# AdaptiveCity/deepdish

Measured on AMD Instinct MI355X. Metric: end-to-end frames/sec (detect+encode+track) at 640x480, higher is better.
Workload: dtype i8 (reference: uint8); encoder f16; 1 GPU; SSD-MobileNet-v1 uint8-quantised (300x300) + MARS-64x32x3 + deep_sort on synthetic 640x480 BGR frames, ~20 synthetic detections/frame (BASELINE.json configs[1]); streams_per_gpu=3072, worker_threads_per_gpu=2, parallelism=independent streams, 3072 per GPU in 2 worker groups, weights=seeded synthetic (seed 1234)

## Files before the change

deepdish_amd/build.py:

```python
import os
import subprocess
import sys
from concurrent.futures import ThreadPoolExecutor

HERE = os.path.dirname(os.path.abspath(__file__))
CSRC = os.path.join(HERE, 'csrc')
OBJ = os.path.join(CSRC, '_obj')
LIB = os.path.join(HERE, 'libdeepdish_hip.so')
HIPCC = os.environ.get('HIPCC', '/opt/rocm/bin/hipcc')
ARCH = 'gfx950'

COMMON = ['--offload-arch=' + ARCH, '-O3', '-fPIC', '-std=c++17', '-Wall', '-Wno-unused-function',
          '-I', os.path.join(HERE, '..', 'include')]
STRICT_FP = {'kalman.hip', 'cost.hip', 'nms.hip', 'tracker.hip', 'lsap.cpp', 'pyset.cpp', 'api.hip', 'image.hip', 'pipeline.hip', 'mog2.hip', 'post.hip'}


EXTRA = ({'netsq.hip': ['-mllvm', '-amdgpu-mfma-vgpr-form'], 'netsq_front.hip': ['-mllvm', '-amdgpu-mfma-vgpr-form'], 'netsq_mid.hip': ['-mllvm', '-amdgpu-mfma-vgpr-form'], 'mars_tail.hip': ['-mllvm', '-amdgpu-mfma-vgpr-form'],
          'mars_pair.hip': ['-mllvm', '-amdgpu-mfma-vgpr-form']}
         if os.environ.get('DD_NO_VGPR_FORM') != '1' else {})


def _sources():
    return sorted(f for f in os.listdir(CSRC) if f.endswith(('.hip', '.cpp')))


def _headers_mtime():
    hs = [os.path.join(CSRC, f) for f in os.listdir(CSRC) if f.endswith('.h')]
    hs.append(os.path.join(HERE, '..', 'include', 'deepdish_hip.h'))
    return max(os.path.getmtime(h) for h in hs)


def _compile(src, force, hmt):
    obj = os.path.join(OBJ, src + '.o')
    path = os.path.join(CSRC, src)
    if (not force and os.path.exists(obj)
            and os.path.getmtime(obj) >= max(os.path.getmtime(path), hmt, os.path.getmtime(__file__))):
        return obj, False
    cmd = [HIPCC] + COMMON + (['-ffp-contract=off'] if src in STRICT_FP else []) + EXTRA.get(src, []) + ['-x', 'hip', '-c', path, '-o', obj]
    r = subprocess.run(cmd, capture_output=True, text=True)
    if r.returncode != 0:
# ... 27 lines not shown
```

deepdish_amd/csrc/net_priv.h:

```cpp
#pragma once
#include <map>
#include <utility>
#include <vector>
#include "common.h"

struct TensorDesc { int buf, h, w, c, cs, coff, dtype, pad; };

struct dd_net {
    dd_ctx *ctx = nullptr;
    int max_batch = 0;
    std::vector<int32_t> prog;
    std::vector<TensorDesc> tensors;
    std::vector<int64_t> buf_elems;
    std::vector<void *> bufs;
    std::vector<int> buf_dtype;
    int n_ops = 0, ops_off = 0;
    void *arena = nullptr;
    int64_t arena_bytes = 0;
    char *d_weights = nullptr;
    int64_t weight_bytes = 0;
    int in_h = 0, in_w = 0, out_tensor = -1;
    bool profile = false;
    int last_batch = 0;
    DevBuf slab;
    bool ssd_dec = false, yolo_dec = false;
    int dec_anchors = 0; float dec_thr = 0.f;
    float *d_anchors = nullptr, *dec_boxes = nullptr, *dec_score = nullptr, *dec_keys = nullptr; int *dec_cls = nullptr;
    bool slab_moved = false;
    _Float16 *d_zero = nullptr;
    bool use_glds = true;
    bool use_rw = true;
    int tile_mode = 0;
    std::vector<hipEvent_t> events;
    std::vector<int32_t> op_launch;
    struct GraphEntry { int calls = 0; hipGraph_t graph = nullptr; hipGraphExec_t exec = nullptr; };
    bool use_graph = false;
    std::map<std::pair<const void *, int>, GraphEntry> graphs;
};

int netq_run_op(dd_net *net, int op_index, const int32_t *o, const uint8_t *input, int nimg, hipStream_t s, int *handled);
int netq_run_front(dd_net *net, const int32_t *o0, const int32_t *o1, const int32_t *o2, const uint8_t *input, int nimg, hipStream_t s, int *ran);
int netq_run_mid(dd_net *net, const int32_t *o3, const int32_t *o4, int nimg, hipStream_t s, int *ran);
int netq_prepare(dd_net *net);
```

deepdish_amd/csrc/nets.hip:

```cpp
#include <algorithm>
#include <cmath>
#include <cstdlib>
#include <map>
#include <string>
#include "common.h"
#include "ssd_dev.h"
#include "net_priv.h"
#include "mars_tail.h"

namespace {

typedef _Float16 h8 __attribute__((ext_vector_type(8)));
typedef _Float16 h4 __attribute__((ext_vector_type(4)));
typedef float f4 __attribute__((ext_vector_type(4)));

enum { OP_INPUT = 1, OP_CONV = 2, OP_DWCONV = 3, OP_MAXPOOL = 4, OP_UPSAMPLE = 5, OP_FC = 6, OP_L2NORM = 7, OP_STEM = 8, OP_DWPW = 9 };
enum { ACT_NONE = 0, ACT_RELU6 = 1, ACT_ELU = 2, ACT_SILU = 3, ACT_RELU = 4, ACT_SIGMOID = 5 };
enum { EPI_F16 = 0, EPI_F32 = 1, EPI_SSD_HEAD = 2, EPI_YOLO = 3 };
enum { OPK_DEFAULT = 0, OPK_FOLDED = 1, OPK_POOL_ROWS = 2, OPK_POOL_ROWS_STEM = 3, OPK_RES_UNIT = 4, OPK_SSD_FRONT = 5, OPK_C64_ROWS = 6, OPK_S2_ROWS = 7, OPK_CONV_WS = 8, OPK_WS_DW = 9, OPK_DWPW_ROWS = 10, OPK_SSD_HEAD_DEC = 11, OPK_RES_PAIR = 12, OPK_YOLO_HEAD_DEC = 13, OPK_MARS_WS = 14, OPK_FOLDED_PREV = 15, OPK_MARS_PAIR = 16, OPK_C64_STRIPS = 18, OPK_Q_FRONT = 19, OPK_Q_MID = 20, OPK_STEM_WIDE = 23 };
enum { DT_F16 = 0, DT_F32 = 1, DT_U8 = 2 };

constexpr int OP_WORDS = 48;
constexpr int TENSOR_WORDS = 8;

__device__ __forceinline__ float fast_sigmoid(float v) { return __builtin_amdgcn_rcpf(1.f + __expf(-v)); }

__device__ __forceinline__ float yolo_box_col(int o, float s, float px, float py, float stride, float aw, float ah, float img_w, float img_h) {
#pragma clang fp contract(off)
    if (o == 0) return (s * 2.f - 0.5f + px) * stride / img_w;
    if (o == 1) return (s * 2.f - 0.5f + py) * stride / img_h;
    if (o == 2) return (s * 2.f) * (s * 2.f) * aw / img_w;
    return (s * 2.f) * (s * 2.f) * ah / img_h;
}

__device__ __forceinline__ float apply_act(float v, int act) {
    switch (act) {
        case ACT_RELU6: return __builtin_amdgcn_fmed3f(v, 0.f, 6.f);
        case ACT_ELU: {
            float e = __builtin_amdgcn_exp2f(v * 1.44269504088896340736f);
            e = __builtin_amdgcn_fmed3f(e, 0.f, 1.f);
            return __builtin_amdgcn_fmed3f(v, e - 1.f, 3.0e38f);
        }
        case ACT_SILU: {
            float r = v * fast_sigmoid(v);
#if defined(__HIP_DEVICE_COMPILE__)
// ... 4324 lines not shown
    bool stem_pending = false;
    bool wide_pending = false, wide_ready = false;
    bool input_pending = false;
    float input_mean = 0.f, input_scale = 1.f;
    int input_op = -1;
    ConvP unit_a;
    bool unit_pending = false;
    ConvP pw_p;
    bool pw_pending = false;
    bool proj_done = false;
    MarsPairP pair64;
    bool pair64_first = false;
    int pair_left = 0;
    ConvP pair_a, pair_b;
    bool pair_pending = false;
    int pair_op = -1;
    auto flush_pair = [&]() -> int {
        pair_pending = false;
        net->op_launch[pair_op] = OPK_RES_UNIT;
        return launch_res_unit(s, pair_a, pair_b, nimg, net->ctx->device);
    };
    auto run_ws = [&](ConvP &P) { return P.cin == 256 ? launch_conv_ws<4>(s, P, net->ctx->device) : launch_conv_ws<8>(s, P, net->ctx->device); };
    int first_op = 0;
    bool mid_on = false;
    {
        static const int chunk_env = getenv("DD_Q_FRONT_CHUNK") ? atoi(getenv("DD_Q_FRONT_CHUNK")) : 0;
        auto opw = [&](int k) { return net->prog.data() + net->ops_off + (size_t)k * OP_WORDS; };
        const char *front_env = getenv("DD_Q_FRONT"), *front_min_env = getenv("DD_Q_FRONT_MIN");
        const int front_min = front_min_env ? atoi(front_min_env) : 24;
        {
            const char *mid_env = getenv("DD_Q_MID");
            mid_on = !(mid_env && atoi(mid_env) == 0) && nimg >= front_min;
        }
        if (!(front_env && atoi(front_env) == 0) && chunk_env <= 0 && nimg >= front_min && net->n_ops > 3 && opw(0)[0] == 16 && opw(1)[0] == 19 && opw(2)[0] == 19) {
            if (net->profile) for (int k = 0; k < 3; ++k) DD_HIP(hipEventRecord(net->events[k], s));
            int ran = 0;
            const int rc = netq_run_front(net, opw(0), opw(1), opw(2), input, nimg, s, &ran);
            if (rc != DD_OK) return rc;
            if (ran) { first_op = 3; net->op_launch[0] = OPK_FOLDED; net->op_launch[1] = OPK_FOLDED; net->op_launch[2] = OPK_Q_FRONT; }
        }
        if (first_op == 0 && chunk_env > 0 && nimg > chunk_env && net->n_ops > 3 && opw(0)[0] == 16 && opw(1)[0] == 19 && opw(2)[0] == 19 && opw(1)[1] == opw(0)[2] && opw(2)[1] == opw(1)[2]) {
            const TensorDesc &t2 = net->tensors[opw(2)[2]];
            const size_t img_out = (size_t)(t2.h + 2) * (t2.w + 2) * t2.cs;
            void *&out_buf = net->bufs[t2.buf];
            void *const out_base = out_buf;
            if (net->profile) for (int k = 0; k < 3; ++k) DD_HIP(hipEventRecord(net->events[k], s));
            for (int c0 = 0; c0 < nimg; c0 += chunk_env) {
                const int nc = std::min(chunk_env, nimg - c0);
                out_buf = static_cast<char *>(out_base) + (size_t)c0 * img_out;
                for (int k = 0; k < 3; ++k) {
                    int handled = 0;
                    const int rc = netq_run_op(net, k, opw(k), input + (size_t)c0 * net->in_h * net->in_w * 3, nc, s, &handled);
                    if (rc != DD_OK || !handled) { out_buf = out_base; return rc != DD_OK ? rc : DD_E_ARG; }
                }
            }
            out_buf = out_base;
            first_op = 3;
        }
    }
    for (int i = first_op; i < net->n_ops; ++i) {
        if (net->profile) DD_HIP(hipEventRecord(net->events[i], s));
        const int32_t *o = net->prog.data() + net->ops_off + (size_t)i * OP_WORDS;
        const float *of = reinterpret_cast<const float *>(o);
        const int kind = o[0], src = o[1], dst = o[2], res = o[3], dst2 = o[4];
        const TensorDesc *ts = src >= 0 ? &net->tensors[src] : nullptr;
        const TensorDesc *td = dst >= 0 ? &net->tensors[dst] : nullptr;
        DD_REQUIRE(!input_pending || (kind == OP_CONV && i == input_op + 1), DD_E_STATE, "dd_net_forward: input op %d was folded into an op that did not take it", input_op);
        if (mid_on && kind == 19 && i + 1 < net->n_ops && net->prog[net->ops_off + (size_t)(i + 1) * OP_WORDS] == 19) {
            const int32_t *o4 = net->prog.data() + net->ops_off + (size_t)(i + 1) * OP_WORDS;
            if (net->profile) DD_HIP(hipEventRecord(net->events[i + 1], s));
            int ran = 0;
            const int rc = netq_run_mid(net, o, o4, nimg, s, &ran);
            if (rc != DD_OK) return rc;
            if (ran) { net->op_launch[i] = OPK_FOLDED; net->op_launch[i + 1] = OPK_Q_MID; ++i; continue; }
        }
        DD_REQUIRE((!wide_pending || kind == OP_CONV) && (!wide_ready || kind == OP_MAXPOOL), DD_E_STATE, "dd_net_forward: op %d does not take the first layer folded into it", i);
        if (pair_pending && kind != OP_CONV) { const int rc = flush_pair(); if (rc != DD_OK) return rc; }
        if (pw_pending && kind != OP_DWCONV) {
            pw_pending = false; net->op_launch[i - 1] = OPK_CONV_WS;
            const int rc = run_ws(pw_p);
            if (rc != DD_OK) return rc;
        }
        if (unit_pending && kind != OP_CONV) {
            unit_pending = false; net->op_launch[i - 1] = OPK_DEFAULT;
            const int rc = launch_conv3x3_rw(s, unit_a, nimg, false, net->ctx->device);
            if (rc != DD_OK) return rc;
        }
        if (stem_pending && !(kind == OP_CONV && o[29]) && kind != OP_DWPW) {
            stem_pending = false; net->op_launch[i - 1] = OPK_DEFAULT;
            const int rc = launch_stem(s, stem_p, nimg);
            if (rc != DD_OK) return rc;
        }
        switch (kind) {
            case OP_INPUT: {
                const int s2d = o[5];
                const int m = nimg * td->h * td->w;
                if (s2d && o[30] && !o[6] && td->cs == 32 && !td->coff && i + 1 < net->n_ops && net->use_rw) {
// ... 403 lines not shown
```

deepdish_amd/csrc/netsq_front.hip:

```cpp
#include <algorithm>
#include <atomic>
#include <cstdlib>
#include <type_traits>
#include "common.h"
#include "net_priv.h"
#include "netsq_dev.h"

namespace {

constexpr int F_S0 = 300, F_S1 = 150, F_S2 = 75;
constexpr int F_PP = (F_S1 + 2) * 16;
constexpr int F_RB0 = 2 * F_PP, F_RB1 = 4 * F_PP;
constexpr int F_NR0 = 4, F_NR1 = 3;
constexpr int F_OP1 = 4 * 320 * 16, F_OP2 = 4 * 80 * 16;
constexpr int F_LDS = F_NR0 * F_RB0 + F_NR1 * F_RB1 + F_OP1 + F_OP2;
constexpr int F_PPO = (F_S2 + 2) * 16;

struct QFrontP {
    const uint8_t *src; long long src_bytes;
    uint8_t *out;
    const i4v *w0, *w0l; const int *cb0; int in_zp, zp0;
    const uint2 *dwa1; const int *dcb1; const i4v *w1; const int *cb1; int zp1;
    const uint2 *dwa2; const int *dcb2; const i4v *w2, *w2l; const int *cb2;
    QReq R0, Rd1, Rp1, Rd2, Rp2;
// ... 261 lines not shown
            __builtin_amdgcn_s_waitcnt(0xc07f);
            __builtin_amdgcn_s_barrier();
            F_STAMP(6);
        }
        g += r_hi - r_lo + 1;
    }
#undef F_STAMP
    if (P.dbg && lane == 0) for (int k = 0; k < 7; ++k) P.dbg[((size_t)blockIdx.x * 4 + wave) * 8 + k] = st[k];
}

}

int netq_run_front(dd_net *net, const int32_t *o0, const int32_t *o1, const int32_t *o2, const uint8_t *input, int nimg, hipStream_t s, int *ran) {
    *ran = 0;
    if (o0[0] != OP_QCONV0 || o1[0] != OP_QDWPW || o2[0] != OP_QDWPW || o1[1] != o0[2] || o2[1] != o1[2]) return DD_OK;
    const TensorDesc &t0 = net->tensors[o0[2]], &t1 = net->tensors[o1[2]], &t2 = net->tensors[o2[2]];
    if (net->in_h != F_S0 || net->in_w != F_S0 || t0.h != F_S1 || t0.w != F_S1 || t0.cs != 32 || t1.h != F_S1 || t1.w != F_S1 || t1.cs != 64 ||
        t2.h != F_S2 || t2.w != F_S2 || t2.cs != 128 || !t0.pad || !t1.pad || !t2.pad) return DD_OK;
    if (o0[7] != 2 || o0[8] != 0 || o0[9] != 0 || o1[7] != 1 || o1[8] != 1 || o1[9] != 1 || o1[10] != 32 || o1[11] != 64 ||
        o2[7] != 2 || o2[8] != 0 || o2[9] != 0 || o2[10] != 64 || o2[11] != 128) return DD_OK;
    const bool split = o0[18] != 0;
    if ((o1[47] != 0) != split || (o2[18] != 0) != split || o0[38] != 0 || o1[38] != 0 || o2[38] != 0 || (!split && o1[18] != 0)) return DD_OK;
    if (!o0[17] || !o1[17] || !o1[21] || !o2[17] || !o2[21] || !o1[20] || !o2[20]) return DD_OK;
    char *W = net->d_weights;
    QFrontP P;
    memset(&P, 0, sizeof(P));
    P.src = input; P.src_bytes = (long long)nimg * F_S0 * F_S0 * 3;
    P.out = static_cast<uint8_t *>(net->bufs[t2.buf]);
    auto blob = [&](int32_t off) { return W + (size_t)(uint32_t)off; };
    P.w0 = reinterpret_cast<const i4v *>(blob(o0[16])); P.w0l = split ? reinterpret_cast<const i4v *>(blob(o0[18])) : nullptr;
    P.cb0 = reinterpret_cast<const int *>(blob(o0[17])); P.in_zp = o0[39]; P.R0 = make_req(o0); P.zp0 = (P.R0.zo ^ 0x80) & 0xff;
    auto dwreq = [&](const int32_t *o) { int32_t d[48] = {0}; d[32] = o[22]; d[33] = o[23]; d[36] = o[24]; d[37] = o[25]; d[40] = o[28]; return make_req(d); };
    P.dwa1 = reinterpret_cast<const uint2 *>(blob(o1[20])); P.dcb1 = reinterpret_cast<const int *>(blob(o1[21]));
    P.w1 = reinterpret_cast<const i4v *>(blob(o1[16])); P.cb1 = reinterpret_cast<const int *>(blob(o1[17]));
    P.Rd1 = dwreq(o1); P.Rp1 = make_req(o1); P.zp1 = (P.Rp1.zo ^ 0x80) & 0xff;
    P.dwa2 = reinterpret_cast<const uint2 *>(blob(o2[20])); P.dcb2 = reinterpret_cast<const int *>(blob(o2[21]));
    P.w2 = reinterpret_cast<const i4v *>(blob(o2[16])); P.w2l = split ? reinterpret_cast<const i4v *>(blob(o2[18])) : nullptr;
    P.cb2 = reinterpret_cast<const int *>(blob(o2[17]));
    P.Rd2 = dwreq(o2); P.Rp2 = make_req(o2);
    const QReq *R[5] = {&P.R0, &P.Rd1, &P.Rp1, &P.Rd2, &P.Rp2};
    bool byte_clamp = true, small_shift = true;
    for (const QReq *r : R) {
        if (r->linear || r->e < 1) return DD_OK;
        byte_clamp = byte_clamp && r->lo == 0 && r->hi == 255;
        small_shift = small_shift && r->e <= 8;
    }
// ... 38 lines not shown
```

deepdish_amd/csrc/netsq_mid.hip:

```cpp
#include <algorithm>
#include <atomic>
#include <cstdlib>
#include <type_traits>
#include "common.h"
#include "net_priv.h"
#include "netsq_dev.h"

namespace {

constexpr int M_S3 = 75, M_S4 = 38;
constexpr int M_PP = (M_S3 + 2) * 16;
constexpr int M_RB = 8 * M_PP;
constexpr int M_NRI = 6, M_NR3 = 3;
constexpr int M_OP3 = 8 * 160 * 16, M_OP4 = 8 * 48 * 16;
constexpr int M_LDS = M_NRI * M_RB + M_NR3 * M_RB + M_OP3 + M_OP4;
constexpr int M_PPO = (M_S4 + 2) * 16;

struct QMidP {
    const uint8_t *in;
    uint8_t *out;
    const uint2 *dwa3; const int *dcb3; const i4v *w3, *w3l; const int *cb3; int zp3;
    const uint2 *dwa4; const int *dcb4; const i4v *w4, *w4l; const int *cb4;
    QReq Rd3, Rp3, Rd4, Rp4;
};
// ... 213 lines not shown
            __builtin_amdgcn_s_barrier();
            if (t + 1 <= r_hi) request_rows(n, 2 * t + 3, 2);
            dw3_stage(t);
            dw4_stage(t);
            __builtin_amdgcn_s_waitcnt(0xc07f);
            __builtin_amdgcn_s_barrier();
        }
        g += r_hi - r_lo + 1;
    }
}

}

int netq_run_mid(dd_net *net, const int32_t *o3, const int32_t *o4, int nimg, hipStream_t s, int *ran) {
    *ran = 0;
    if (o3[0] != OP_QDWPW || o4[0] != OP_QDWPW || o4[1] != o3[2] || o3[1] < 0) return DD_OK;
    const TensorDesc &ti = net->tensors[o3[1]], &t3 = net->tensors[o3[2]], &t4 = net->tensors[o4[2]];
    if (ti.h != M_S3 || ti.w != M_S3 || ti.cs != 128 || t3.h != M_S3 || t3.w != M_S3 || t3.cs != 128 || t4.h != M_S4 || t4.w != M_S4 || t4.cs != 256 ||
        !ti.pad || !t3.pad || !t4.pad) return DD_OK;
    if (o3[7] != 1 || o3[8] != 1 || o3[9] != 1 || o3[10] != 128 || o3[11] != 128 || o4[7] != 2 || o4[8] != 1 || o4[9] != 1 || o4[10] != 128 || o4[11] != 256) return DD_OK;
    const bool split = o3[18] != 0;
    if ((o4[18] != 0) != split || o3[38] != 0 || o4[38] != 0 || o3[47] != 0 || o4[47] != 0) return DD_OK;
    if (!o3[17] || !o3[20] || !o3[21] || !o4[17] || !o4[20] || !o4[21]) return DD_OK;
    char *W = net->d_weights;
    QMidP P;
    memset(&P, 0, sizeof(P));
    P.in = static_cast<const uint8_t *>(net->bufs[ti.buf]);
    P.out = static_cast<uint8_t *>(net->bufs[t4.buf]);
    auto blob = [&](int32_t off) { return W + (size_t)(uint32_t)off; };
    auto dwreq = [&](const int32_t *o) { int32_t d[48] = {0}; d[32] = o[22]; d[33] = o[23]; d[36] = o[24]; d[37] = o[25]; d[40] = o[28]; return make_req(d); };
    P.dwa3 = reinterpret_cast<const uint2 *>(blob(o3[20])); P.dcb3 = reinterpret_cast<const int *>(blob(o3[21]));
    P.w3 = reinterpret_cast<const i4v *>(blob(o3[16])); P.w3l = split ? reinterpret_cast<const i4v *>(blob(o3[18])) : nullptr;
    P.cb3 = reinterpret_cast<const int *>(blob(o3[17])); P.Rd3 = dwreq(o3); P.Rp3 = make_req(o3); P.zp3 = (P.Rp3.zo ^ 0x80) & 0xff;
    P.dwa4 = reinterpret_cast<const uint2 *>(blob(o4[20])); P.dcb4 = reinterpret_cast<const int *>(blob(o4[21]));
    P.w4 = reinterpret_cast<const i4v *>(blob(o4[16])); P.w4l = split ? reinterpret_cast<const i4v *>(blob(o4[18])) : nullptr;
    P.cb4 = reinterpret_cast<const int *>(blob(o4[17])); P.Rd4 = dwreq(o4); P.Rp4 = make_req(o4);
    const QReq *R[4] = {&P.Rd3, &P.Rp3, &P.Rd4, &P.Rp4};
    bool byte_clamp = true, small_shift = true;
    for (const QReq *r : R) {
        if (r->linear || r->e < 1) return DD_OK;
        byte_clamp = byte_clamp && r->lo == 0 && r->hi == 255;
        small_shift = small_shift && r->e <= 8;
    }
    const int sat = byte_clamp ? (small_shift ? 2 : 1) : 0;
    void (*kern)(const QMidP, const int, const int) =
        split ? (sat == 2 ? &q_mid_k<2, true> : sat == 1 ? &q_mid_k<1, true> : &q_mid_k<0, true>)
// ... 19 lines not shown
```

deepdish_amd/netsq.py:

```python
import os
import numpy as np

from . import nets, quantize
from .nets import Program, same_pad, DT_U8

OP_QCONV0, OP_QCONV, OP_QDW, OP_QDWPW, OP_QSSD_DECODE, OP_QADD = 16, 17, 18, 19, 20, 21
QEPI_Q16, QEPI_ROWS, QEPI_Q16N = 0, 1, 2
FUSE_BLOCKS = os.environ.get('DD_Q_FUSE', '1') != '0'
ADD_FUSE = os.environ.get('DD_Q_ADD_FUSE', '1') != '0'
SPLIT_PW = os.environ.get('DD_Q_SPLIT_PW', '1') != '0'
SPLIT_PW_MAX_CIN = int(os.environ.get('DD_Q_SPLIT_PW_MAX_CIN', '128'))
SPLIT_PW_MIN_CIN = int(os.environ.get('DD_Q_SPLIT_PW_MIN_CIN', '64'))
DUP32 = os.environ.get('DD_Q_DUP32', '1') != '0'
MERGE_HEADS = os.environ.get('DD_Q_MERGE_HEADS', '1') != '0'
FUSED_SHAPES = {(32, 64, 1), (64, 128, 2), (128, 128, 1), (128, 256, 2), (256, 256, 1), (256, 512, 2), (512, 512, 1)}
FEATURE_LAYERS = ['pw11', 'pw13', 'extra1_2', 'extra2_2', 'extra3_2', 'extra4_2']


def _req_words(L):
    m, shift = quantize.conv_multiplier(L)
    if shift > 0:
        raise ValueError('uint8 layer with a multiplier >= 1 (shift %d): not built' % shift)
    lo, hi = quantize.activation_range(L)
    linear = int(L['act'] == 'none')
# ... 204 lines not shown
        wp, cb, kcpt = pack_conv(Lp, QEPI_Q16)
        zwc = 128 - int(Lp['w_zp'])
        w_lo = 0
        dup = 0
        if DUP32 and cin == 32 and zwc != 0:
            x = Lp['w'].astype(np.int64) - int(Lp['w_zp'])
            hi = np.clip(x, -128, 127)
            if (x - hi).max() <= 127:
                wp, _, kcpt = pack_conv(dict(Lp, w=np.concatenate([hi + 128, x - hi + 128], axis=2).astype(np.int64)), QEPI_Q16)
                cb = (Lp['bias'].astype(np.int64) + (128 - int(Lp['in_zp'])) * x.reshape(cin, cout).sum(axis=0)).astype(np.int32)
                zwc, dup = 0, 1
        if SPLIT_PW and SPLIT_PW_MIN_CIN <= cin <= SPLIT_PW_MAX_CIN and zwc != 0:
            x = Lp['w'].astype(np.int64) - int(Lp['w_zp'])
            hi = np.clip(x, -128, 127)
            if (x - hi).max() <= 127:
                wp, _, _ = pack_conv(dict(Lp, w=(hi + 128).astype(np.int64)), QEPI_Q16)
                wl, _, _ = pack_conv(dict(Lp, w=(x - hi + 128).astype(np.int64)), QEPI_Q16)
                w_lo = P.add_blob(wl)
                cb = (Lp['bias'].astype(np.int64) + (128 - int(Lp['in_zp'])) * x.reshape(cin, cout).sum(axis=0)).astype(np.int32)
                zwc = 0
        dst = P.qtensor(ho, wo, cout, Lp['out_zp'])
        raw = dict(rp)
        raw.update({38: zwc, 39: int(Lp['in_zp']), 45: P.add_blob(folded_addends(dcb, rd)), 46: P.add_blob(folded_addends(cb, rp)), 47: dup})
        P._op(OP_QDWPW, src=src, dst=dst, kh=1, kw=1, stride=stride, pad_t=pt, pad_l=pl, cin=cin, cout=cout, cout_pad=cout, kpad=kcpt,
              w_off=P.add_blob(wp), b_off=P.add_blob(cb), aff_off=w_lo, ho=ho, wo=wo,
              p=[P.add_blob(dwa), P.add_blob(dcb), rd[32], rd[33], rd[36], rd[37]], bk=rd[40], raw=raw)
        info('q_dwpw_k', 2 * ho * wo * cin * (9 + cout), s['h'] * s['w'] * cin + ho * wo * cout, cin * (9 + cout) + 4 * (cin + cout), s['h'] * s['w'] * cin)
        return dst

    feats = {}
    for i in range(1, 14):
        x = dwpw(x, f'dw{i}', f'pw{i}')
        feats[f'pw{i}'] = x
    for j in range(1, 5):
        x = conv(conv(x, f'extra{j}_1'), f'extra{j}_2')
        feats[f'extra{j}_2'] = x
    n_cls = Ls['cls0']['w'].shape[3] // nets.SSD_ANCHORS_PER_MAP[0]
    cls_row = (n_cls + 15) // 16 * 16
    box_t = P.tensor(n_anchors, 1, 4, cs=4, dtype=DT_U8)
    cls_t = P.tensor(n_anchors, 1, n_cls, cs=cls_row, dtype=DT_U8)
    base = 0
    for k, (fname, a) in enumerate(zip(FEATURE_LAYERS, nets.SSD_ANCHORS_PER_MAP)):
        ft = feats[fname]
        fm = P.T(ft)['h']
        _model_need(fm == maps[k], 'feature map %d is %dx%d (the anchors are laid out for %d)' % (k, fm, fm, maps[k]))
        for other in (f'box{k}', f'cls{k}'):
# ... 199 lines not shown
```

deepdish_amd/profile.py:

```python
import ctypes
import numpy as np

from ._lib import lib, check
from .runtime import ptr

PEAK_F16_TFLOPS = 2500.0
PEAK_HBM_GBS = 8000.0
PEAK_I8_TOPS = 5000.0


def last_batch(net):
    n = ctypes.c_int()
    check(lib().dd_net_last_batch(net._h, ctypes.byref(n)), 'dd_net_last_batch')
    return n.value


def net_op_times(net):
    n = len(net.program.ops)
    ms = np.zeros(n, dtype=np.float32)
    cnt = ctypes.c_int()
    check(lib().dd_net_profile_read(net._h, ptr(ms), n, ctypes.byref(cnt)), 'dd_net_profile_read')
    return ms


OPK_FOLDED = 1
OPK_NAMES = {2: 'conv3x3_pool_rows_k', 3: 'conv3x3_pool_rows_k<STEM>', 4: 'res_unit_rows_k', 5: 'ssd_front_k', 6: 'conv3x3_c64_rows_k', 7: 'conv3x3_s2_rows_k', 8: 'conv_ws_k', 9: 'conv_ws_dw_k', 10: 'dwpw_rows_k', 11: 'conv_glds_k<ssd_head_decode>', 12: 'res_pair_rows_k', 13: 'conv_glds_k<yolo_head_decode>', 14: 'mars_ws128_k', 16: 'mars_pair64_k', 17: 'q_dwm_k', 18: 'conv3x3_c64_rows_k<strips>', 19: 'q_front_k', 20: 'q_mid_k', 21: 'q_conv_k<add>', 22: 'q_add_k', 23: 'stem_conv_pool_wide_k'}
OPK_FOLDED_PREV = 15


def net_op_launches(net):
    n = len(net.program.ops)
    codes = np.zeros(n, dtype=np.int32)
    cnt = ctypes.c_int(0)
    check(lib().dd_net_op_launches(net._h, ptr(codes), n, ctypes.byref(cnt)), 'dd_net_op_launches')
    return codes


def launches_of(net, ms, batch):
    out, pend = [], None
    for t, info, code in zip(ms, net.program.info, net_op_launches(net)):
        fl, by = info['flops'] * batch, info['bytes'] * batch + info.get('wbytes', 0)
        if code == OPK_FOLDED:
            if pend is None:
                pend = [float(t), fl, info.get('src_bytes', 0) * batch + info.get('wbytes', 0)]
            else:
                pend[0] += float(t); pend[1] += fl; pend[2] += info.get('wbytes', 0)
            continue
        if code == OPK_FOLDED_PREV and out:
            k0, t0, f0, b0 = out[-1]
# ... 87 lines not shown
```

Before: 144,400 frames/s.

## Fuse late quantised 38x38 and stride-2 dw+pw layer pair into one kernel

Adds a q_late_k kernel that runs two consecutive quantised depthwise+pointwise layers (38x38x256 stride 1, then stride 2 to 19x19x512) in a single persistent launch. The intermediate activation stays in LDS rings and is never written to HBM, which cuts one launch and one round-trip of intermediate memory traffic. The packer also emits a hi/lo split weight form for zero-point-weighted cin=256 layers so the fused path applies to them. A guard keeps the fused path, and the existing front and mid fusions, off when a later op still reads the skipped intermediate tensor. The costs are a large LDS footprint, one block per CU, and extra MFMA work for the split weights.

```diff
diff --git a/deepdish_amd/build.py b/deepdish_amd/build.py
--- a/deepdish_amd/build.py
+++ b/deepdish_amd/build.py
@@ -15,7 +15,8 @@
 STRICT_FP = {'kalman.hip', 'cost.hip', 'nms.hip', 'tracker.hip', 'lsap.cpp', 'pyset.cpp', 'api.hip', 'image.hip', 'pipeline.hip', 'mog2.hip', 'post.hip'}
 
 
-EXTRA = ({'netsq.hip': ['-mllvm', '-amdgpu-mfma-vgpr-form'], 'netsq_front.hip': ['-mllvm', '-amdgpu-mfma-vgpr-form'], 'netsq_mid.hip': ['-mllvm', '-amdgpu-mfma-vgpr-form'], 'mars_tail.hip': ['-mllvm', '-amdgpu-mfma-vgpr-form'],
+EXTRA = ({'netsq.hip': ['-mllvm', '-amdgpu-mfma-vgpr-form'], 'netsq_front.hip': ['-mllvm', '-amdgpu-mfma-vgpr-form'], 'netsq_mid.hip': ['-mllvm', '-amdgpu-mfma-vgpr-form'], 'netsq_late.hip': ['-mllvm', '-amdgpu-mfma-vgpr-form'],
+          'mars_tail.hip': ['-mllvm', '-amdgpu-mfma-vgpr-form'],
           'mars_pair.hip': ['-mllvm', '-amdgpu-mfma-vgpr-form']}
          if os.environ.get('DD_NO_VGPR_FORM') != '1' else {})
 
diff --git a/deepdish_amd/csrc/net_priv.h b/deepdish_amd/csrc/net_priv.h
--- a/deepdish_amd/csrc/net_priv.h
+++ b/deepdish_amd/csrc/net_priv.h
@@ -38,7 +38,17 @@
     std::map<std::pair<const void *, int>, GraphEntry> graphs;
 };
 
+constexpr int NET_OP_WORDS = 48;
+
+inline bool net_tensor_read_behind(const dd_net *net, const int32_t *last, int t) {
+    const int32_t *const end = net->prog.data() + net->ops_off + (size_t)net->n_ops * NET_OP_WORDS;
+    for (const int32_t *o = last + NET_OP_WORDS; o < end; o += NET_OP_WORDS)
+        if (o[1] == t || o[3] == t || o[4] == t) return true;
+    return false;
+}
+
 int netq_run_op(dd_net *net, int op_index, const int32_t *o, const uint8_t *input, int nimg, hipStream_t s, int *handled);
 int netq_run_front(dd_net *net, const int32_t *o0, const int32_t *o1, const int32_t *o2, const uint8_t *input, int nimg, hipStream_t s, int *ran);
 int netq_run_mid(dd_net *net, const int32_t *o3, const int32_t *o4, int nimg, hipStream_t s, int *ran);
+int netq_run_late(dd_net *net, const int32_t *o5, const int32_t *o6, int nimg, hipStream_t s, int *ran);
 int netq_prepare(dd_net *net);
diff --git a/deepdish_amd/csrc/nets.hip b/deepdish_amd/csrc/nets.hip
--- a/deepdish_amd/csrc/nets.hip
+++ b/deepdish_amd/csrc/nets.hip
@@ -17,10 +17,11 @@
 enum { OP_INPUT = 1, OP_CONV = 2, OP_DWCONV = 3, OP_MAXPOOL = 4, OP_UPSAMPLE = 5, OP_FC = 6, OP_L2NORM = 7, OP_STEM = 8, OP_DWPW = 9 };
 enum { ACT_NONE = 0, ACT_RELU6 = 1, ACT_ELU = 2, ACT_SILU = 3, ACT_RELU = 4, ACT_SIGMOID = 5 };
 enum { EPI_F16 = 0, EPI_F32 = 1, EPI_SSD_HEAD = 2, EPI_YOLO = 3 };
-enum { OPK_DEFAULT = 0, OPK_FOLDED = 1, OPK_POOL_ROWS = 2, OPK_POOL_ROWS_STEM = 3, OPK_RES_UNIT = 4, OPK_SSD_FRONT = 5, OPK_C64_ROWS = 6, OPK_S2_ROWS = 7, OPK_CONV_WS = 8, OPK_WS_DW = 9, OPK_DWPW_ROWS = 10, OPK_SSD_HEAD_DEC = 11, OPK_RES_PAIR = 12, OPK_YOLO_HEAD_DEC = 13, OPK_MARS_WS = 14, OPK_FOLDED_PREV = 15, OPK_MARS_PAIR = 16, OPK_C64_STRIPS = 18, OPK_Q_FRONT = 19, OPK_Q_MID = 20, OPK_STEM_WIDE = 23 };
+enum { OPK_DEFAULT = 0, OPK_FOLDED = 1, OPK_POOL_ROWS = 2, OPK_POOL_ROWS_STEM = 3, OPK_RES_UNIT = 4, OPK_SSD_FRONT = 5, OPK_C64_ROWS = 6, OPK_S2_ROWS = 7, OPK_CONV_WS = 8, OPK_WS_DW = 9, OPK_DWPW_ROWS = 10, OPK_SSD_HEAD_DEC = 11, OPK_RES_PAIR = 12, OPK_YOLO_HEAD_DEC = 13, OPK_MARS_WS = 14, OPK_FOLDED_PREV = 15, OPK_MARS_PAIR = 16, OPK_C64_STRIPS = 18, OPK_Q_FRONT = 19, OPK_Q_MID = 20, OPK_STEM_WIDE = 23, OPK_Q_LATE = 24 };
 enum { DT_F16 = 0, DT_F32 = 1, DT_U8 = 2 };
 
 constexpr int OP_WORDS = 48;
+static_assert(OP_WORDS == NET_OP_WORDS, "csrc/net_priv.h walks the op records too");
 constexpr int TENSOR_WORDS = 8;
 
 __device__ __forceinline__ float fast_sigmoid(float v) { return __builtin_amdgcn_rcpf(1.f + __expf(-v)); }
@@ -4391,7 +4392,7 @@
     };
     auto run_ws = [&](ConvP &P) { return P.cin == 256 ? launch_conv_ws<4>(s, P, net->ctx->device) : launch_conv_ws<8>(s, P, net->ctx->device); };
     int first_op = 0;
-    bool mid_on = false;
+    bool mid_on = false, late_on = false;
     {
         static const int chunk_env = getenv("DD_Q_FRONT_CHUNK") ? atoi(getenv("DD_Q_FRONT_CHUNK")) : 0;
         auto opw = [&](int k) { return net->prog.data() + net->ops_off + (size_t)k * OP_WORDS; };
@@ -4400,6 +4401,8 @@
         {
             const char *mid_env = getenv("DD_Q_MID");
             mid_on = !(mid_env && atoi(mid_env) == 0) && nimg >= front_min;
+            const char *late_env = getenv("DD_Q_LATE");
+            late_on = !(late_env && atoi(late_env) == 0) && nimg >= front_min;
         }
         if (!(front_env && atoi(front_env) == 0) && chunk_env <= 0 && nimg >= front_min && net->n_ops > 3 && opw(0)[0] == 16 && opw(1)[0] == 19 && opw(2)[0] == 19) {
             if (net->profile) for (int k = 0; k < 3; ++k) DD_HIP(hipEventRecord(net->events[k], s));
@@ -4435,13 +4438,21 @@
         const TensorDesc *ts = src >= 0 ? &net->tensors[src] : nullptr;
         const TensorDesc *td = dst >= 0 ? &net->tensors[dst] : nullptr;
         DD_REQUIRE(!input_pending || (kind == OP_CONV && i == input_op + 1), DD_E_STATE, "dd_net_forward: input op %d was folded into an op that did not take it", input_op);
-        if (mid_on && kind == 19 && i + 1 < net->n_ops && net->prog[net->ops_off + (size_t)(i + 1) * OP_WORDS] == 19) {
+        if ((mid_on || late_on) && kind == 19 && i + 1 < net->n_ops && net->prog[net->ops_off + (size_t)(i + 1) * OP_WORDS] == 19) {
             const int32_t *o4 = net->prog.data() + net->ops_off + (size_t)(i + 1) * OP_WORDS;
             if (net->profile) DD_HIP(hipEventRecord(net->events[i + 1], s));
             int ran = 0;
-            const int rc = netq_run_mid(net, o, o4, nimg, s, &ran);
-            if (rc != DD_OK) return rc;
-            if (ran) { net->op_launch[i] = OPK_FOLDED; net->op_launch[i + 1] = OPK_Q_MID; ++i; continue; }
+            if (mid_on) {
+                const int rc = netq_run_mid(net, o, o4, nimg, s, &ran);
+                if (rc != DD_OK) return rc;
+                if (ran) net->op_launch[i + 1] = OPK_Q_MID;
+            }
+            if (!ran && late_on) {
+                const int rc = netq_run_late(net, o, o4, nimg, s, &ran);
+                if (rc != DD_OK) return rc;
+                if (ran) net->op_launch[i + 1] = OPK_Q_LATE;
+            }
+            if (ran) { net->op_launch[i] = OPK_FOLDED; ++i; continue; }
         }
         DD_REQUIRE((!wide_pending || kind == OP_CONV) && (!wide_ready || kind == OP_MAXPOOL), DD_E_STATE, "dd_net_forward: op %d does not take the first layer folded into it", i);
         if (pair_pending && kind != OP_CONV) { const int rc = flush_pair(); if (rc != DD_OK) return rc; }
diff --git a/deepdish_amd/csrc/netsq_front.hip b/deepdish_amd/csrc/netsq_front.hip
--- a/deepdish_amd/csrc/netsq_front.hip
+++ b/deepdish_amd/csrc/netsq_front.hip
@@ -307,6 +307,7 @@
     const bool split = o0[18] != 0;
     if ((o1[47] != 0) != split || (o2[18] != 0) != split || o0[38] != 0 || o1[38] != 0 || o2[38] != 0 || (!split && o1[18] != 0)) return DD_OK;
     if (!o0[17] || !o1[17] || !o1[21] || !o2[17] || !o2[21] || !o1[20] || !o2[20]) return DD_OK;
+    if (net_tensor_read_behind(net, o2, o0[2]) || net_tensor_read_behind(net, o2, o1[2])) return DD_OK;
     char *W = net->d_weights;
     QFrontP P;
     memset(&P, 0, sizeof(P));
diff --git a/deepdish_amd/csrc/netsq_late.hip b/deepdish_amd/csrc/netsq_late.hip
--- /dev/null
+++ b/deepdish_amd/csrc/netsq_late.hip
@@ -0,0 +1,346 @@
+#include <algorithm>
+#include <atomic>
+#include <cstdlib>
+#include <type_traits>
+#include "common.h"
+#include "net_priv.h"
+#include "netsq_dev.h"
+
+namespace {
+
+constexpr int L_S5 = 38, L_S6 = 19;
+constexpr int L_VR = L_S5 + 1;
+constexpr int L_PP = (L_S5 + 2) * 16;
+constexpr int L_RB = 16 * L_PP;
+constexpr int L_NRI = 8, L_NR5 = 4;
+constexpr int L_OP5 = 16 * 96 * 16, L_OP6 = 16 * 32 * 16;
+constexpr int L_CB = (256 + 512 + 256 + 256) * 4;
+constexpr int L_LDS = L_NRI * L_RB + L_NR5 * L_RB + L_OP5 + L_OP6 + L_CB;
+constexpr int L_PPO = (L_S6 + 2) * 16;
+
+struct QLateP {
+    const uint8_t *in;
+    uint8_t *out;
+    const uint2 *dwa5; const int *dcb5; const i4v *w5, *w5l; const int *cb5; int zp5;
+    const uint2 *dwa6; const int *dcb6; const i4v *w6, *w6l; const int *cb6;
+    QReq Rd5, Rp5, Rd6, Rp6;
+};
+
+template <int SAT, bool SPLIT>
+__global__ __launch_bounds__(1024) void q_late_k(const QLateP P, const int rows_total, const int rows_per_block) {
+    extern __shared__ __attribute__((aligned(16))) uint8_t smem[];
+    uint8_t *const ring_in = smem;
+    uint8_t *const ring5 = ring_in + L_NRI * L_RB;
+    uint8_t *const opnd5 = ring5 + L_NR5 * L_RB;
+    uint8_t *const opnd6 = opnd5 + L_OP5;
+    int *const cbl = reinterpret_cast<int *>(opnd6 + L_OP6);
+    const int tid = threadIdx.x, lane = tid & 63, wave = __builtin_amdgcn_readfirstlane(tid >> 6);
+    const int fr = lane & 15, fq = lane >> 4;
+    const int g_begin = blockIdx.x * rows_per_block, g_end = min(rows_total, g_begin + rows_per_block);
+    if (g_begin >= g_end) return;
+
+    unsigned dmask[4];
+#pragma unroll
+    for (int d = 0; d < 4; ++d) dmask[d] = (fr >> 2) == d ? 0xffu << (8 * (fr & 3)) : 0u;
+    int tap_dx[3];
+#pragma unroll
+    for (int ks = 0; ks < 3; ++ks) tap_dx[ks] = (min(4 * ks + fq, 8) % 3) * 16;
+    const bool row_up0 = fq == 3, row_up1 = fq >= 2;
+    auto build_a = [&](const unsigned w, i4v (&A)[3]) {
+#pragma unroll
+        for (int ks = 0; ks < 3; ++ks) {
+            const unsigned rh = __builtin_amdgcn_perm(w, w, 0x01010101u * (unsigned)ks);
+#pragma unroll
+            for (int d = 0; d < 4; ++d) A[ks][d] = (int)(rh & dmask[d]);
+        }
+    };
+    i4v A5h[3], A6h[3];
+    const uint2 ab5 = P.dwa5[wave * 64 + lane], ab6 = P.dwa6[wave * 64 + lane];
+    build_a(ab5.x, A5h);
+    build_a(ab6.x, A6h);
+    const unsigned lom5 = (unsigned)__builtin_amdgcn_readfirstlane((int)(ab5.y >> 24));
+    const unsigned lom6 = (unsigned)__builtin_amdgcn_readfirstlane((int)(ab6.y >> 24));
+    for (int i = tid; i < 256; i += 1024) { cbl[i] = P.cb5[i]; cbl[768 + i] = P.dcb5[i]; cbl[1024 + i] = P.dcb6[i]; }
+    for (int i = tid; i < 512; i += 1024) cbl[256 + i] = P.cb6[i];
+    const i4v *const dcb5 = reinterpret_cast<const i4v *>(cbl + 768 + 16 * wave + 4 * fq);
+    const i4v *const dcb6 = reinterpret_cast<const i4v *>(cbl + 1024 + 16 * wave + 4 * fq);
+    i4v W5[4], W6[2][4];
+    unsigned nz5 = 0, nz6 = 0;
+#pragma unroll
+    for (int kc = 0; kc < 4; ++kc) {
+        W5[kc] = P.w5[(wave * 4 + kc) * 64 + lane];
+        if constexpr (SPLIT) {
+            const i4v a = P.w5l[(wave * 4 + kc) * 64 + lane];
+            if (__builtin_amdgcn_ballot_w64((a[0] | a[1] | a[2] | a[3]) != 0) != 0ull) nz5 |= 1u << kc;
+        }
+#pragma unroll
+        for (int m = 0; m < 2; ++m) {
+            W6[m][kc] = P.w6[((wave * 2 + m) * 4 + kc) * 64 + lane];
+            if constexpr (SPLIT) {
+                const i4v b = P.w6l[((wave * 2 + m) * 4 + kc) * 64 + lane];
+                if (__builtin_amdgcn_ballot_w64((b[0] | b[1] | b[2] | b[3]) != 0) != 0ull) nz6 |= 1u << (m * 4 + kc);
+            }
+        }
+    }
+    const i4v *const cb5 = reinterpret_cast<const i4v *>(cbl + 64 * (wave >> 2) + 16 * fq + 4 * (wave & 3));
+    const i4v *const cb6 = reinterpret_cast<const i4v *>(cbl + 256 + 64 * (wave >> 1) + 16 * fq + 8 * (wave & 1));
+    const int Md5 = P.Rd5.M, shd5 = P.Rd5.e - 1, lod5 = P.Rd5.lo, hid5 = P.Rd5.hi;
+    const int Mp5 = P.Rp5.M, shp5 = P.Rp5.e - 1, lop5 = P.Rp5.lo, hip5 = P.Rp5.hi;
+    const int Md6 = P.Rd6.M, shd6 = P.Rd6.e - 1, lod6 = P.Rd6.lo, hid6 = P.Rd6.hi;
+    const int Mp6 = P.Rp6.M, shp6 = P.Rp6.e - 1, lop6 = P.Rp6.lo, hip6 = P.Rp6.hi;
+    const long long Cd5 = q_signed_c<SAT>(P.Rd5.C, shd5), Cp5 = q_signed_c<SAT>(P.Rp5.C, shp5), Cd6 = q_signed_c<SAT>(P.Rd6.C, shd6), Cp6 = q_signed_c<SAT>(P.Rp6.C, shp6);
+    const u4v z5v = {(unsigned)P.zp5 * 0x01010101u, (unsigned)P.zp5 * 0x01010101u, (unsigned)P.zp5 * 0x01010101u, (unsigned)P.zp5 * 0x01010101u};
+
+    for (int i = tid * 16; i < L_NR5 * L_RB; i += 1024 * 16) *reinterpret_cast<u4v *>(ring5 + i) = z5v;
+    __syncthreads();
+
+    const int n0 = g_begin / L_S6, r0 = g_begin - n0 * L_S6;
+    const int n1 = (g_end - 1) / L_S6, r1 = (g_end - 1) - n1 * L_S6;
+    const int G_lo = n0 * L_VR + 2 * r0, G_hi = n1 * L_VR + 2 * r1 + 2;
+
+    auto glds16 = [&](const uint8_t *g, const uint8_t *l) {
+        unsigned keep;
+        const unsigned dst = (unsigned)(uintptr_t)(const __attribute__((address_space(3))) uint8_t *)l;
+        asm volatile("s_mov_b32 %0, m0\n\ts_mov_b32 m0, %2\n\ts_nop 0\n\tglobal_load_lds_dwordx4 %1, off\n\ts_mov_b32 m0, %0"
+                     : "=&s"(keep) : "v"(g), "s"(dst) : "memory");
+    };
+    auto request_rows = [&](int b_from, int b_to) {
+        for (int p = wave; p < 10 * (b_to - b_from + 1); p += 16) {
+            const int rr = p / 10, piece = p - rr * 10, B = b_from + rr;
+            glds16(P.in + (size_t)B * L_RB + (size_t)(piece * 1024 + lane * 16), ring_in + (B & (L_NRI - 1)) * L_RB + piece * 1024);
+        }
+    };
+    auto src_hi = [&](int G) { const int n = G / L_VR, v = min(G - n * L_VR, L_S5 - 1); return n * (L_S5 + 2) + v + 2; };
+
+    auto dw_run = [&](auto nf_tag, const uint8_t *ring, int s0, int s1, int s2, int lane_col, int frag_pitch, const i4v (&Ah)[3], const uint2 *al,
+                      const unsigned lom, const i4v *cbp, int Md, long long Cd, int shd, int lod, int hid, uint8_t *tile) __attribute__((always_inline)) {
+        constexpr int NF = decltype(nf_tag)::value;
+        constexpr int DW_W = 3;
+        const uint8_t *const a0 = ring + (row_up0 ? s1 : s0) + tap_dx[0] + lane_col;
+        const uint8_t *const a1 = ring + (row_up1 ? s2 : s1) + tap_dx[1] + lane_col;
+        const uint8_t *const a2 = ring + s2 + tap_dx[2] + lane_col;
+        i4v acc[NF], b[DW_W];
+        const i4v cb = *cbp;
+        auto opnd_at = [&](int j) __attribute__((always_inline)) { const int ks = j / NF, f = j - ks * NF; return *reinterpret_cast<const i4v *>((ks == 0 ? a0 : ks == 1 ? a1 : a2) + f * frag_pitch); };
+#pragma unroll
+        for (int j = 0; j < DW_W; ++j) b[j] = opnd_at(j);
+#pragma unroll
+        for (int j = 0; j < 3 * NF; ++j) {
+            const int ks = j / NF, f = j - ks * NF;
+            if (ks == 0) acc[f] = __builtin_amdgcn_mfma_i32_16x16x64_i8(Ah[0], b[j % DW_W], cb, 0, 0, 0);
+            else acc[f] = __builtin_amdgcn_mfma_i32_16x16x64_i8(Ah[ks], b[j % DW_W], acc[f], 0, 0, 0);
+            if (j + DW_W < 3 * NF) b[j % DW_W] = opnd_at(j + DW_W);
+        }
+        if (lom) {
+#pragma unroll
+            for (int ks = 0; ks < 3; ++ks) {
+                if (lom & (1u << ks)) {
+                    int li = lane;
+                    asm volatile("" : "+v"(li));
+                    const unsigned lw = al[li].y;
+                    const unsigned rl = __builtin_amdgcn_perm(lw, lw, 0x01010101u * (unsigned)ks);
+                    i4v Al;
+#pragma unroll
+                    for (int d = 0; d < 4; ++d) Al[d] = (int)(rl & (((li >> 2) & 3) == d ? 0xffu << (8 * (li & 3)) : 0u));
+#pragma unroll
+                    for (int f = 0; f < NF; ++f) acc[f] = __builtin_amdgcn_mfma_i32_16x16x64_i8(Al, opnd_at(ks * NF + f), acc[f], 0, 0, 0);
+                }
+            }
+        }
+#pragma unroll
+        for (int f = 0; f < NF; ++f)
+            *reinterpret_cast<unsigned *>(tile + f * 256) = q_requant_pack4s<SAT>(acc[f][0], acc[f][1], acc[f][2], acc[f][3], Md, Cd, Cd, Cd, Cd, shd, lod, hid);
+    };
+    auto dw5_stage = [&](int T) __attribute__((always_inline)) {
+#pragma unroll 1
+        for (int j = 0; j < 2; ++j) {
+            const int G = 2 * T + 1 + j;
+            if (G < G_lo || G > G_hi) continue;
+            const int n = G / L_VR, v = G - n * L_VR;
+            if (v == L_S5) continue;
+            const int B = n * (L_S5 + 2) + v;
+            const int s0 = (B & (L_NRI - 1)) * L_RB + wave * L_PP, s1 = ((B + 1) & (L_NRI - 1)) * L_RB + wave * L_PP, s2 = ((B + 2) & (L_NRI - 1)) * L_RB + wave * L_PP;
+            dw_run(std::integral_constant<int, 3>{}, ring_in, s0, s1, s2, fr * 16, 256, A5h, P.dwa5 + wave * 64, lom5, dcb5, Md5, Cd5, shd5, lod5, hid5,
+                   opnd5 + ((wave * 96 + j * 48 + fr) * 16 + 4 * fq));
+        }
+    };
+    auto dw6_stage = [&](int T) __attribute__((always_inline)) {
+        int c = 2 * T;
+        if (c < 2) return -1;
+        int n = c / L_VR, v = c - n * L_VR;
+        if (v & 1) { c -= 1; v -= 1; }
+        else if (v == 0) { c -= 1; n -= 1; v = L_S5; }
+        if (v < 2) return -1;
+        const int g = n * L_S6 + (v >> 1) - 1;
+        if (g < g_begin || g >= g_end) return -1;
+        const int s0 = ((c - 2) & (L_NR5 - 1)) * L_RB + wave * L_PP, s1 = ((c - 1) & (L_NR5 - 1)) * L_RB + wave * L_PP, s2 = (c & (L_NR5 - 1)) * L_RB + wave * L_PP;
+        dw_run(std::integral_constant<int, 2>{}, ring5, s0, s1, s2, fr * 32 + 16, 512, A6h, P.dwa6 + wave * 64, lom6, dcb6, Md6, Cd6, shd6, lod6, hid6,
+               opnd6 + ((wave * 32 + fr) * 16 + 4 * fq));
+        return g;
+    };
+    auto pw5_stage = [&](int T) __attribute__((always_inline)) {
+#pragma unroll 1
+        for (int j = 0; j < 2; ++j) {
+            const int G = 2 * T - 1 + j;
+            if (G < G_lo || G > G_hi) continue;
+            const int n = G / L_VR, v = G - n * L_VR;
+            uint8_t *const dst = ring5 + (G & (L_NR5 - 1)) * L_RB;
+            if (v == L_S5) {
+                if (lane < L_S5 + 2) *reinterpret_cast<u4v *>(dst + wave * L_PP + lane * 16) = z5v;
+                continue;
+            }
+            const uint8_t *const bp = opnd5 + (fq * 96 + j * 48 + fr) * 16;
+            i4v b[3], acc[3];
+            const i4v cb = *cb5;
+#pragma unroll
+            for (int kc = 0; kc < 4; ++kc) {
+#pragma unroll
+                for (int f = 0; f < 3; ++f) b[f] = *reinterpret_cast<const i4v *>(bp + kc * (4 * 96 * 16) + f * 256);
+#pragma unroll
+                for (int f = 0; f < 3; ++f) acc[f] = __builtin_amdgcn_mfma_i32_16x16x64_i8(W5[kc], b[f], kc == 0 ? cb : acc[f], 0, 0, 0);
+            }
+            if (nz5) {
+#pragma unroll
+                for (int kc = 0; kc < 4; ++kc) {
+                    if (nz5 & (1u << kc)) {
+                        int li = lane;
+                        asm volatile("" : "+v"(li));
+                        const i4v wl = P.w5l[(wave * 4 + kc) * 64 + li];
+#pragma unroll
+                        for (int f = 0; f < 3; ++f) acc[f] = __builtin_amdgcn_mfma_i32_16x16x64_i8(wl, *reinterpret_cast<const i4v *>(bp + kc * (4 * 96 * 16) + f * 256), acc[f], 0, 0, 0);
+                    }
+                }
+            }
+            uint8_t *const d4 = dst + (4 * (wave >> 2) + fq) * L_PP + 4 * (wave & 3) + (fr + 1) * 16;
+#pragma unroll
+            for (int f = 0; f < 3; ++f) {
+                const unsigned o = q_requant_pack4s<SAT>(acc[f][0], acc[f][1], acc[f][2], acc[f][3], Mp5, Cp5, Cp5, Cp5, Cp5, shp5, lop5, hip5);
+                if (f < 2 || fr < 6) *reinterpret_cast<unsigned *>(d4 + f * 256) = o;
+            }
+        }
+    };
+    auto pw6_stage = [&](int g) __attribute__((always_inline)) {
+        if (g < 0) return;
+        const int n = g / L_S6, r = g - n * L_S6;
+        const uint8_t *const bp = opnd6 + (fq * 32 + fr) * 16;
+#pragma unroll
+        for (int m = 0; m < 2; ++m) {
+            if (m) __builtin_amdgcn_sched_barrier(0);
+            i4v b[2], acc[2];
+            const i4v cb = cb6[m];
+#pragma unroll
+            for (int kc = 0; kc < 4; ++kc) {
+#pragma unroll
+                for (int f = 0; f < 2; ++f) b[f] = *reinterpret_cast<const i4v *>(bp + kc * (4 * 32 * 16) + f * 256);
+#pragma unroll
+                for (int f = 0; f < 2; ++f) acc[f] = __builtin_amdgcn_mfma_i32_16x16x64_i8(W6[m][kc], b[f], kc == 0 ? cb : acc[f], 0, 0, 0);
+            }
+            if (nz6 & (0xfu << (4 * m))) {
+#pragma unroll
+                for (int kc = 0; kc < 4; ++kc) {
+                    if (nz6 & (1u << (m * 4 + kc))) {
+                        int li = lane;
+                        asm volatile("" : "+v"(li));
+                        const i4v wl = P.w6l[((wave * 2 + m) * 4 + kc) * 64 + li];
+#pragma unroll
+                        for (int f = 0; f < 2; ++f) acc[f] = __builtin_amdgcn_mfma_i32_16x16x64_i8(wl, *reinterpret_cast<const i4v *>(bp + kc * (4 * 32 * 16) + f * 256), acc[f], 0, 0, 0);
+                    }
+                }
+            }
+            const int c = 2 * wave + m;
+            uint8_t *const dst = P.out + ((size_t)((n * (L_S6 + 2) + r + 1) * 32 + 4 * (c >> 2) + fq) * L_PPO + 4 * (c & 3) + (fr + 1) * 16);
+#pragma unroll
+            for (int f = 0; f < 2; ++f) {
+                const unsigned o = q_requant_pack4s<SAT>(acc[f][0], acc[f][1], acc[f][2], acc[f][3], Mp6, Cp6, Cp6, Cp6, Cp6, shp6, lop6, hip6);
+                if (f < 1 || fr < 3) *reinterpret_cast<unsigned *>(dst + f * 256) = o;
+            }
+        }
+    };
+
+    const int T0 = (G_lo + 1) / 2 - 1, T1 = (G_hi + 1) / 2 + 1;
+    int b_next = n0 * (L_S5 + 2) + 2 * r0;
+    {
+        const int hi = src_hi(min(2 * T0 + 2, G_hi));
+        request_rows(b_next, hi);
+        b_next = hi + 1;
+    }
+    asm volatile("s_waitcnt vmcnt(0)" ::: "memory");
+    __syncthreads();
+    int g6 = -1;
+    for (int T = T0; T <= T1; ++T) {
+        pw5_stage(T);
+        pw6_stage(g6);
+        asm volatile("s_waitcnt vmcnt(0) lgkmcnt(0)" ::: "memory");
+        __builtin_amdgcn_s_barrier();
+        {
+            const int hi = src_hi(min(2 * T + 4, G_hi));
+            if (hi >= b_next) { request_rows(b_next, hi); b_next = hi + 1; }
+        }
+        dw5_stage(T);
+        g6 = dw6_stage(T);
+        __builtin_amdgcn_s_waitcnt(0xc07f);
+        __builtin_amdgcn_s_barrier();
+    }
+}
+
+}
+
+int netq_run_late(dd_net *net, const int32_t *o5, const int32_t *o6, int nimg, hipStream_t s, int *ran) {
+    *ran = 0;
+    if (o5[0] != OP_QDWPW || o6[0] != OP_QDWPW || o6[1] != o5[2] || o5[1] < 0) return DD_OK;
+    const TensorDesc &ti = net->tensors[o5[1]], &t5 = net->tensors[o5[2]], &t6 = net->tensors[o6[2]];
+    if (ti.h != L_S5 || ti.w != L_S5 || ti.cs != 256 || t5.h != L_S5 || t5.w != L_S5 || t5.cs != 256 || t6.h != L_S6 || t6.w != L_S6 || t6.cs != 512 ||
+        !ti.pad || !t5.pad || !t6.pad) return DD_OK;
+    if (o5[7] != 1 || o5[8] != 1 || o5[9] != 1 || o5[10] != 256 || o5[11] != 256 || o6[7] != 2 || o6[8] != 0 || o6[9] != 0 || o6[10] != 256 || o6[11] != 512) return DD_OK;
+    auto split_form = [](const int32_t *o, int32_t &w, int32_t &wl, int32_t &cb) {
+        if (o[38] == 0) { w = o[16]; wl = o[18]; cb = o[17]; return true; }
+        w = o[42]; wl = o[43]; cb = o[44];
+        return w != 0 && wl != 0 && cb != 0;
+    };
+    int32_t w5, w5l, c5, w6, w6l, c6;
+    if (!split_form(o5, w5, w5l, c5) || !split_form(o6, w6, w6l, c6)) return DD_OK;
+    const bool split = w5l != 0;
+    if ((w6l != 0) != split || o5[47] != 0 || o6[47] != 0) return DD_OK;
+    if (!w5 || !c5 || !o5[20] || !o5[21] || !w6 || !c6 || !o6[20] || !o6[21]) return DD_OK;
+    if (net_tensor_read_behind(net, o6, o5[2])) return DD_OK;
+    char *W = net->d_weights;
+    QLateP P;
+    memset(&P, 0, sizeof(P));
+    P.in = static_cast<const uint8_t *>(net->bufs[ti.buf]);
+    P.out = static_cast<uint8_t *>(net->bufs[t6.buf]);
+    auto blob = [&](int32_t off) { return W + (size_t)(uint32_t)off; };
+    auto dwreq = [&](const int32_t *o) { int32_t d[48] = {0}; d[32] = o[22]; d[33] = o[23]; d[36] = o[24]; d[37] = o[25]; d[40] = o[28]; return make_req(d); };
+    P.dwa5 = reinterpret_cast<const uint2 *>(blob(o5[20])); P.dcb5 = reinterpret_cast<const int *>(blob(o5[21]));
+    P.w5 = reinterpret_cast<const i4v *>(blob(w5)); P.w5l = split ? reinterpret_cast<const i4v *>(blob(w5l)) : nullptr;
+    P.cb5 = reinterpret_cast<const int *>(blob(c5)); P.Rd5 = dwreq(o5); P.Rp5 = make_req(o5); P.zp5 = (P.Rp5.zo ^ 0x80) & 0xff;
+    P.dwa6 = reinterpret_cast<const uint2 *>(blob(o6[20])); P.dcb6 = reinterpret_cast<const int *>(blob(o6[21]));
+    P.w6 = reinterpret_cast<const i4v *>(blob(w6)); P.w6l = split ? reinterpret_cast<const i4v *>(blob(w6l)) : nullptr;
+    P.cb6 = reinterpret_cast<const int *>(blob(c6)); P.Rd6 = dwreq(o6); P.Rp6 = make_req(o6);
+    const QReq *R[4] = {&P.Rd5, &P.Rp5, &P.Rd6, &P.Rp6};
+    bool byte_clamp = true, small_shift = true;
+    for (const QReq *r : R) {
+        if (r->linear || r->e < 1) return DD_OK;
+        byte_clamp = byte_clamp && r->lo == 0 && r->hi == 255;
+        small_shift = small_shift && r->e <= 8;
+    }
+    const int sat = byte_clamp ? (small_shift ? 2 : 1) : 0;
+    void (*kern)(const QLateP, const int, const int) =
+        split ? (sat == 2 ? &q_late_k<2, true> : sat == 1 ? &q_late_k<1, true> : &q_late_k<0, true>)
+              : (sat == 2 ? &q_late_k<2, false> : sat == 1 ? &q_late_k<1, false> : &q_late_k<0, false>);
+    static DevOnce once;
+    const int rc = once.run(net->ctx->device, [&]() -> int {
+        for (const void *f : {reinterpret_cast<const void *>(&q_late_k<2, true>), reinterpret_cast<const void *>(&q_late_k<1, true>), reinterpret_cast<const void *>(&q_late_k<0, true>),
+                              reinterpret_cast<const void *>(&q_late_k<2, false>), reinterpret_cast<const void *>(&q_late_k<1, false>), reinterpret_cast<const void *>(&q_late_k<0, false>)})
+            DD_HIP(hipFuncSetAttribute(f, hipFuncAttributeMaxDynamicSharedMemorySize, L_LDS));
+        return DD_OK;
+    });
+    if (rc != DD_OK) return rc;
+    const int n_cu = dd_cu_count(net->ctx->device);
+    const int rows_total = nimg * L_S6;
+    const int blocks = std::max(1, std::min(n_cu, rows_total / 8));
+    const int rpb = dd_ceil_div(rows_total, blocks);
+    hipLaunchKernelGGL(kern, dim3((unsigned)dd_ceil_div(rows_total, rpb)), dim3(1024), L_LDS, s, P, rows_total, rpb);
+    DD_LAUNCH_CHECK();
+    *ran = 1;
+    return DD_OK;
+}
diff --git a/deepdish_amd/csrc/netsq_mid.hip b/deepdish_amd/csrc/netsq_mid.hip
--- a/deepdish_amd/csrc/netsq_mid.hip
+++ b/deepdish_amd/csrc/netsq_mid.hip
@@ -259,6 +259,7 @@
     const bool split = o3[18] != 0;
     if ((o4[18] != 0) != split || o3[38] != 0 || o4[38] != 0 || o3[47] != 0 || o4[47] != 0) return DD_OK;
     if (!o3[17] || !o3[20] || !o3[21] || !o4[17] || !o4[20] || !o4[21]) return DD_OK;
+    if (net_tensor_read_behind(net, o4, o3[2])) return DD_OK;
     char *W = net->d_weights;
     QMidP P;
     memset(&P, 0, sizeof(P));
diff --git a/deepdish_amd/netsq.py b/deepdish_amd/netsq.py
--- a/deepdish_amd/netsq.py
+++ b/deepdish_amd/netsq.py
@@ -250,6 +250,14 @@
         dst = P.qtensor(ho, wo, cout, Lp['out_zp'])
         raw = dict(rp)
         raw.update({38: zwc, 39: int(Lp['in_zp']), 45: P.add_blob(folded_addends(dcb, rd)), 46: P.add_blob(folded_addends(cb, rp)), 47: dup})
+        if zwc != 0 and cin == 256:
+            x = Lp['w'].astype(np.int64) - int(Lp['w_zp'])
+            hi = np.clip(x, -128, 127)
+            if (x - hi).max() <= 127:
+                wh, _, _ = pack_conv(dict(Lp, w=(hi + 128).astype(np.int64)), QEPI_Q16)
+                wl, _, _ = pack_conv(dict(Lp, w=(x - hi + 128).astype(np.int64)), QEPI_Q16)
+                cbs = (Lp['bias'].astype(np.int64) + (128 - int(Lp['in_zp'])) * x.reshape(cin, cout).sum(axis=0)).astype(np.int32)
+                raw.update({42: P.add_blob(wh), 43: P.add_blob(wl), 44: P.add_blob(cbs)})
         P._op(OP_QDWPW, src=src, dst=dst, kh=1, kw=1, stride=stride, pad_t=pt, pad_l=pl, cin=cin, cout=cout, cout_pad=cout, kpad=kcpt,
               w_off=P.add_blob(wp), b_off=P.add_blob(cb), aff_off=w_lo, ho=ho, wo=wo,
               p=[P.add_blob(dwa), P.add_blob(dcb), rd[32], rd[33], rd[36], rd[37]], bk=rd[40], raw=raw)
diff --git a/deepdish_amd/profile.py b/deepdish_amd/profile.py
--- a/deepdish_amd/profile.py
+++ b/deepdish_amd/profile.py
@@ -24,7 +24,7 @@
 
 
 OPK_FOLDED = 1
-OPK_NAMES = {2: 'conv3x3_pool_rows_k', 3: 'conv3x3_pool_rows_k<STEM>', 4: 'res_unit_rows_k', 5: 'ssd_front_k', 6: 'conv3x3_c64_rows_k', 7: 'conv3x3_s2_rows_k', 8: 'conv_ws_k', 9: 'conv_ws_dw_k', 10: 'dwpw_rows_k', 11: 'conv_glds_k<ssd_head_decode>', 12: 'res_pair_rows_k', 13: 'conv_glds_k<yolo_head_decode>', 14: 'mars_ws128_k', 16: 'mars_pair64_k', 17: 'q_dwm_k', 18: 'conv3x3_c64_rows_k<strips>', 19: 'q_front_k', 20: 'q_mid_k', 21: 'q_conv_k<add>', 22: 'q_add_k', 23: 'stem_conv_pool_wide_k'}
+OPK_NAMES = {2: 'conv3x3_pool_rows_k', 3: 'conv3x3_pool_rows_k<STEM>', 4: 'res_unit_rows_k', 5: 'ssd_front_k', 6: 'conv3x3_c64_rows_k', 7: 'conv3x3_s2_rows_k', 8: 'conv_ws_k', 9: 'conv_ws_dw_k', 10: 'dwpw_rows_k', 11: 'conv_glds_k<ssd_head_decode>', 12: 'res_pair_rows_k', 13: 'conv_glds_k<yolo_head_decode>', 14: 'mars_ws128_k', 16: 'mars_pair64_k', 17: 'q_dwm_k', 18: 'conv3x3_c64_rows_k<strips>', 19: 'q_front_k', 20: 'q_mid_k', 21: 'q_conv_k<add>', 22: 'q_add_k', 23: 'stem_conv_pool_wide_k', 24: 'q_late_k'}
 OPK_FOLDED_PREV = 15
 
 
```

New measurement: 144,500 frames/s (median of 2 runs). Within noise of the previous version (+0.1%).
